# Beinsezii/skrample

Hardware: AMD Instinct MI355X
Metric: sampler steps/sec (fused DPM-2 SDE step, eps-pred, Karras sigmas, Bx4x128x128 bf16) + achieved HBM GB/s (higher is better)
Workload: dtype f32; 1 GPU; DPM order-2 SDE (eta=1) + Karras(Scaled) sigmas, eps-pred, B=256x4x128x128 bf16 latents per GPU (BASELINE north-star shape; cfg2 at 4x batch), in-kernel Philox noise, one fused launch per step; global_batch=256, per_gpu_batch=256, latent_dtype=bf16, compute_dtype=f32 registers, fp64 host coefficients, schedule_steps=20, buffer_sets=7, buffer_set_bytes=167772160, precondition_steps=3000, parallelism=batch-shard x1, no collective

## Files before the change

include/skrample_hip.h:

```cpp
#ifndef SKRAMPLE_HIP_H
#define SKRAMPLE_HIP_H

#include <stdint.h>

#ifdef __cplusplus
extern "C" {
#endif

#define SKR_ABI_VERSION 15
#define SKR_MAX_TERMS 80


enum skr_status {
  SKR_OK = 0,
  SKR_ERR_NULL = 1,
  SKR_ERR_DTYPE = 2,
  SKR_ERR_TERMS = 3,
  SKR_ERR_ALIGN = 4,
  SKR_ERR_SHAPE = 5,
  SKR_ERR_LAUNCH = 6,
  SKR_ERR_UNSUPPORTED = 7,
  SKR_ERR_LIBRARY = 8,
  SKR_ERR_CAPTURE = 9,
};

enum skr_dtype { SKR_BF16 = 0, SKR_F16 = 1, SKR_F32 = 2, SKR_F64 = 3, SKR_NONE = -1 };

typedef struct skr_step_plan {
  int32_t n_terms;
  int32_t n_group_a;
  int32_t dtype_a;
  int32_t dtype_b;
  int32_t out0_dtype;
  int32_t out1_dtype;
  int32_t acc_f64;
  int32_t noise_mode;
  double coef0[SKR_MAX_TERMS];
  double coef1[SKR_MAX_TERMS];
  double chain;
  double zeta0, zeta1;
  uint64_t stream0, stream1;
  int64_t sample_numel;
// ... 289 lines not shown
```

skrample_amd/_hip.py:

```python

from __future__ import annotations

import ctypes
import operator
import os
import sys
import threading

import torch

MAX_TERMS = 80
ABI_VERSION = 15
SKR_ERR_UNSUPPORTED = 7

BF16, F16, F32, F64, NONE = 0, 1, 2, 3, -1
DTYPE_CODE = {torch.bfloat16: BF16, torch.float16: F16, torch.float32: F32, torch.float64: F64}
CODE_DTYPE = {v: k for k, v in DTYPE_CODE.items()}

LIB_NAME = "libskrample_hip.so"
LIB_PATH = os.environ.get("SKR_HIP_LIB") or os.path.join(os.path.dirname(os.path.abspath(__file__)), "csrc", LIB_NAME)

EXPORTS = (
    "skr_step_launch",
    "skr_step_launch_indexed",
    "skr_step_launch_indexed_per_sample",
    "skr_step_launch_rolling",
    "skr_step_launch_channels_last",
    "skr_step_launch_masked",
# ... 689 lines not shown
```

skrample_amd/csrc/skr_step.hip:

```cpp


#include "skr_device.h"
#include "skr_step_common.h"
#include <new>

namespace skr {

Tuning g_tune;

template <typename T, typename Acc, bool HAS1, int N, int UV, bool TILE>
__device__ __forceinline__ void acc_batch(const StepArgs<Acc>& a, int k, int64_t v0, int64_t vhi, Acc s0[UV][VEC], Acc s1[UV][VEC]) {
  Raw<T> raw[UV][N];
#pragma unroll
  for (int u = 0; u < UV; ++u) {
    const int64_t v = v0 + u * BLOCK;
    if (v < vhi) {
#pragma unroll
      for (int j = 0; j < N; ++j) raw[u][j] = load_raw<T, TILE>(a.in[k + j], v);
    }
  }
#pragma unroll
  for (int u = 0; u < UV; ++u) {
    if (v0 + u * BLOCK >= vhi) continue;
#pragma unroll
// ... 226 lines not shown
        s1[i] = fma_(a.c1[1], ov[i], fma_(a.c1[0], sv[i], 0.f));
      }
#pragma unroll
      for (int j = 2; j < K; ++j) {
        float w[VEC];
        widen<T, float>(raw[u][j], w);
        const float c = a.c1[j];
#pragma unroll
        for (int i = 0; i < VEC; ++i) s1[i] = fma_(c, w[i], s1[i]);
      }
#pragma unroll
      for (int i = 0; i < VEC; ++i) s1[i] = fma_(a.chain, d[i], s1[i]);
      store8<T, float, TILE>(a.out1, v, s1);
      store8<T, float, TILE>(a.out0, v, d);
    }
  }
}


struct Geometry { dim3 grid; int mode; };

template <int UV, bool NOISE>
static Geometry geometry(int64_t numel, int64_t sample_numel) {
  const int64_t nvec = numel / VEC, per_block = BLOCK * UV;
  const bool aligned = (sample_numel % VEC) == 0;
  const int64_t vps = sample_numel / VEC, batch = numel / sample_numel;
  if (NOISE && aligned && vps >= per_block / 2 && batch <= 65535ll * 65535ll) {
    int64_t bx = (vps + per_block - 1) / per_block;
    if (bx > 65535) bx = 65535;
    const int64_t gy = batch < 65535 ? batch : 65535;
// ... 61 lines not shown
  Geometry g = geometry<UV, false>(args.numel, args.sample_numel);
  RkArgs ra;
  fill_operands(args.in, args.c1, args.n_terms, ra.in, ra.c1);
  ra.out0 = args.out0; ra.out1 = args.out1; ra.chain = args.chain;
  for (int i = 0; i < 4; ++i) ra.ck[i] = (float)args.ck[i];
  ra.conv_to = args.conv_to; ra.conv_from = args.conv_from; ra.numel = args.numel;
  return with_tile<sizeof(T) == 4>(args.numel, args.sample_numel, false, g.mode, [&](auto tile) {
    with_count<2, 8>(args.n_terms, [&](auto n) {
      hipLaunchKernelGGL((step_kernel_rk<T, decltype(n)::value, UV, decltype(tile)::value>), g.grid, dim3(BLOCK), 0, stream, ra);
    });
    return finish_launch();
  });
}

template <typename T>
static int launch_rk(const StepArgs<float>& args, hipStream_t stream) {
  {
    bool taken = false;
    const int rc = launch_one_trip_rk<T>(args, false, stream, taken);
    if (taken) return rc;
  }
  if (has_table(args.form)) return SKR_ERR_UNSUPPORTED;
  const int uv = g_tune.rk_uv ? g_tune.rk_uv : 1;
  if (uv == 4) return launch_rk_uv<T, 4>(args, stream);
  if (uv == 2) return launch_rk_uv<T, 2>(args, stream);
  return launch_rk_uv<T, 1>(args, stream);
}

template <typename TA, typename TB, typename TO0, typename TO1, typename Acc, bool ST0, bool HAS1, bool NOISE, bool CONV>
static int launch(StepArgs<Acc>& args, hipStream_t stream) {
  if constexpr (std::is_same<Acc, float>::value && std::is_same<TA, TB>::value && std::is_same<TO0, TA>::value && ST0 && !HAS1 && !CONV) {
    if (args.n_a == args.n_terms && (!NOISE || args.zeta0 != 0.f || has_table(args.form))) {
      bool taken = false;
      const int rc = launch_k<TA, NOISE>(args, stream, taken);
      if (taken) return rc;
    }
  }
  if constexpr (std::is_same<Acc, float>::value && std::is_same<TA, TB>::value && std::is_same<TO0, TA>::value && std::is_same<TO1, TA>::value && ST0 && HAS1 && CONV) {
    if (args.n_terms >= 2 && args.n_terms <= 8 && args.numel % VEC == 0) {
      if constexpr (!NOISE) return launch_rk<TA>(args, stream);
      else {
        bool taken = false;
        const int rc = launch_one_trip_rk<TA>(args, true, stream, taken);
        if (taken) return rc;
      }
    }
  }
  if constexpr (std::is_same<Acc, float>::value && sizeof(TA) == 2 && (std::is_same<TB, TA>::value || std::is_same<TB, float>::value) &&
                std::is_same<TO0, float>::value && std::is_same<TO1, TA>::value && ST0 && HAS1 && !CONV) {
    bool taken = false;
    const int rc = launch_one_trip_two<TA>(args, NOISE, std::is_same<TB, float>::value, stream, taken);
    if (taken) return rc;
  }
  if (has_table(args.form)) return SKR_ERR_UNSUPPORTED;
  constexpr int UV = uv_for(NOISE, HAS1);
  Geometry g = geometry<UV, NOISE>(args.numel, args.sample_numel);
  args.grid_mode = g.mode;
  args.vps = args.sample_numel / VEC;
  constexpr bool HAS32 = std::is_same<Acc, float>::value && (std::is_same<TA, float>::value || std::is_same<TB, float>::value ||
                                                               (ST0 && std::is_same<TO0, float>::value) || (HAS1 && std::is_same<TO1, float>::value));
  return with_tile<HAS32>(args.numel, args.sample_numel, NOISE, g.mode, [&](auto tile) {
    hipLaunchKernelGGL((step_kernel<TA, TB, TO0, TO1, Acc, ST0, HAS1, NOISE, CONV, decltype(tile)::value>), g.grid, dim3(BLOCK), 0, stream, args);
// ... 43 lines not shown
    a.c1[k] = (Acc)p.coef1[k];
  }
  for (int k = p.n_terms; k < MAXK; ++k) { a.in[k] = nullptr; a.c0[k] = 0; a.c1[k] = 0; }
  a.out0 = out0; a.out1 = out1; a.seeds = seeds;
  a.chain = (Acc)p.chain; a.zeta0 = (Acc)p.zeta0; a.zeta1 = (Acc)p.zeta1;
  a.stream0 = p.stream0; a.stream1 = p.stream1;
  a.numel = numel;
  a.sample_numel = p.sample_numel > 0 ? p.sample_numel : (numel > 0 ? numel : 1);
  a.inv_sample_numel = 1.0 / (double)a.sample_numel;
  a.n_a = p.n_group_a; a.n_terms = p.n_terms;
  a.conv_to = p.convert_to; a.conv_from = p.convert_from;
  for (int i = 0; i < 4; ++i) a.ck[i] = p.convert_k[i];
  if (a.conv_to != 0 || a.conv_from != 0) {
    for (int k = 0; k < p.n_terms; ++k) a.c0[k] = 0;
  }
  return pick<Acc>(a, p, s);
}

}

using skr::aligned16;

static int samples_ok(const skr_step_plan& p, int64_t numel, int64_t multiple) {
  if (p.sample_numel <= 0 || numel % p.sample_numel != 0) return SKR_ERR_SHAPE;
  return p.sample_numel % multiple == 0 ? SKR_OK : SKR_ERR_UNSUPPORTED;
}

static int validate_plan(const skr_step_plan& p, int64_t numel) {
  if (p.n_terms < 0 || p.n_terms > SKR_MAX_TERMS || p.n_group_a < 0 || p.n_group_a > p.n_terms) return SKR_ERR_TERMS;
  if (numel < 0) return SKR_ERR_SHAPE;
  if (p.out0_dtype == SKR_NONE && p.out1_dtype == SKR_NONE) return SKR_ERR_NULL;
  if (p.noise_mode != 0 && p.noise_mode != 1) return SKR_ERR_UNSUPPORTED;
  if (p.convert_to < 0 || p.convert_to > 3 || p.convert_from < 0 || p.convert_from > 3) return SKR_ERR_UNSUPPORTED;
  if ((p.convert_to || p.convert_from) && (p.n_group_a < 2 || p.out1_dtype == SKR_NONE)) return SKR_ERR_TERMS;
  if (skr::plan_draws(p) && numel > 0) return samples_ok(p, numel, 8);
  return SKR_OK;
}

int skr::step_launch_checks(const skr_step_plan* plan, const void* const* inputs, void* out0, void* out1, const uint64_t* seeds_dev, int64_t numel,
                            skr::RowForm form, const skr_step_row* rows, const int32_t* index, bool& empty) {
  empty = false;
  if (!plan || (has_table(form) && (!rows || (per_sample_rows(form) && !index)))) return SKR_ERR_NULL;
  const skr_step_plan& p = *plan;
  if (p.noise_mode == 1 && (has_table(form) || skr::plan_draws(p)) && numel > 0 && !seeds_dev) return SKR_ERR_NULL;
  if (const int rc = validate_plan(p, numel)) return rc;
  if (numel == 0) { empty = true; return SKR_OK; }
  const bool st0 = p.out0_dtype != SKR_NONE, has1 = p.out1_dtype != SKR_NONE;
  if ((p.n_terms > 0 && !inputs) || (st0 && !out0) || (has1 && !out1)) return SKR_ERR_NULL;
  if (const int rc = skr::check_ptrs(inputs, p.n_terms)) return rc;
// ... 3 lines not shown

static int step_launch_impl(const skr_step_plan* plan, const void* const* inputs, void* out0, void* out1, const uint64_t* seeds_dev, int64_t numel,
                            void* stream, skr::RowForm form, const skr_step_row* rows, const int32_t* index, int32_t row_offset) {
  skr::DeviceGuard device_guard(out0 ? out0 : out1);
  bool empty = false;
  if (const int rc = skr::step_launch_checks(plan, inputs, out0, out1, seeds_dev, numel, form, rows, index, empty)) return rc;
  if (empty) return SKR_OK;
  const skr_step_plan& p = *plan;
  hipStream_t s = reinterpret_cast<hipStream_t>(stream);
  if (has_table(form)) {
    const bool ragged = skr::ragged_launch(p, numel, form);
    if (per_sample_rows(form) || p.noise_mode == 1) {
      const int rc = samples_ok(p, numel, per_sample_rows(form) ? 2048 : 8);
      if (rc != SKR_OK && !(ragged && rc == SKR_ERR_UNSUPPORTED)) return rc;
    }
    if (p.acc_f64 || p.n_terms > SKR_ROW_TERMS || row_offset < 0) return SKR_ERR_UNSUPPORTED;
    if (ragged) return skr::launch_ragged(p, inputs, out0, seeds_dev, numel, s, form, rows, index, row_offset);
    return skr::run<float>(p, inputs, out0, out1, seeds_dev, numel, s, form, rows, index, row_offset);
  }
  return p.acc_f64 ? skr::run<double>(p, inputs, out0, out1, seeds_dev, numel, s)
                   : skr::run<float>(p, inputs, out0, out1, seeds_dev, numel, s);
}

extern "C" int skr_step_launch(const skr_step_plan* plan, const void* const* inputs, void* out0, void* out1,
                               const uint64_t* seeds_dev, int64_t numel, void* stream) {
  return step_launch_impl(plan, inputs, out0, out1, seeds_dev, numel, stream, skr::RowForm::Kernarg, nullptr, nullptr, 0);
}

extern "C" int skr_step_launch_indexed(const skr_step_plan* plan, const void* const* inputs, void* out0, void* out1,
                                       const uint64_t* seeds_dev, int64_t numel, const skr_step_row* rows_dev,
                                       const int32_t* index_dev, int32_t row_offset, void* stream) {
// ... 72 lines not shown
```

skrample_amd/csrc/skr_step_common.h:

```cpp
#pragma once
#include <hip/hip_runtime.h>
#include <stdlib.h>
#include <stdint.h>
#include <string.h>
#include <type_traits>
#include "../../include/skrample_hip.h"
#include "skr_philox.h"
#include "skr_pack.h"
#include "skr_launch.h"

namespace skr {

struct Tuning {
  int one_trip, xmap, tile, rk_uv, two_out, pace, rk_blk, two_nt, tape_words;
  Tuning() {
    const char* e;
    one_trip = !((e = getenv("SKR_ONE_TRIP")) && e[0] == '0');
    xmap = (e = getenv("SKR_XMAP")) ? atoi(e) : 7;
    tile = getenv("SKR_NO_TILE") == nullptr;
    rk_uv = (e = getenv("SKR_RK_UV")) ? atoi(e) : 0;
    two_out = getenv("SKR_NO_TWO_OUT") == nullptr;
    pace = getenv("SKR_NO_PACE") == nullptr;
    two_nt = (e = getenv("SKR_TWO_NT")) ? atoi(e) : -1;
    rk_blk = (e = getenv("SKR_RK_BLK")) ? atoi(e) : 0;
// ... 336 lines not shown
__device__ __forceinline__ void fma_noise8(Acc zeta, const float z[VEC], Acc s[VEC]) {
#pragma unroll
  for (int i = 0; i < VEC; ++i) s[i] = fma_(zeta, (Acc)z[i], s[i]);
}

struct RkArgs {
  const void* in[8];
  float c1[8];
  void* out0;
  void* out1;
  float chain;
  float ck[4];
  int32_t conv_to, conv_from;
  int64_t numel;
};

__device__ __forceinline__ uint32_t chunk_of(uint32_t b, int lr) {
  const uint32_t g = 3 + lr;
  return ((b >> g) << g) + ((b & 7u) << lr) + ((b >> 3) & ((1u << lr) - 1u));
}

static inline int xmap_lr_for(int64_t chunks) {
  int lr = g_tune.xmap;
  if (lr < 0) lr = 0;
  if (lr > 20) lr = 20;
  while (lr > 0 && chunks % (8ll << lr) != 0) --lr;
  return lr;
}

extern thread_local int g_last_hip_error;
// ... 40 lines not shown
```

skrample_amd/csrc/skr_step_fast.hip:

```cpp
#include "skr_step_common.h"

namespace skr {

template <int KMAX>
struct OneTripArgs {
  const void* in[KMAX];
  void* out0;
  const uint64_t* seeds;
  int32_t xmap_lr;
  int32_t bps_shift;
  uint64_t stream0;
  float c0[KMAX];
  float zeta0;
  RowRef tab;
};



template <bool PER_SAMPLE>
__device__ __forceinline__ const skr_step_row* row_at(const RowRef& r, uint32_t c, int32_t bps_shift) {
  if constexpr (PER_SAMPLE) {
    const uint32_t smp = (c >> (bps_shift < 0 ? 0 : bps_shift)) / (bps_shift < 0 ? (uint32_t)(-bps_shift) : 1u);
    return r.rows + ((r.index != nullptr ? r.index[__builtin_amdgcn_readfirstlane(smp)] : 0) + r.row_offset);
  } else {
// ... 252 lines not shown
  for (int j = 2; j < K; ++j) {
    if constexpr (F == RowForm::Rolling) { if (!on[j]) continue; }
    float w[VEC];
    widen<T, float>(raw[j], w);
    const float cj = cf[j];
#pragma unroll
    for (int i = 0; i < VEC; ++i) s1[i] = fma_(cj, w[i], s1[i]);
  }
#pragma unroll
  for (int i = 0; i < VEC; ++i) s1[i] = fma_(chain, d[i], s1[i]);
  if constexpr (NOISE) { if (n1) fma_noise8<float>(zeta1, z1, s1); }
  store8<T, float, TILE>(a.out1, v, s1);
  store8<T, float, TILE>(a.out0, v, d);
}

static bool one_trip_ok(int64_t numel, int64_t sample_numel, bool noise, RowForm form, int* bps_shift) {
  constexpr int64_t CHUNK = (int64_t)BLOCK * VEC;
  if ((!g_tune.one_trip && !has_table(form)) || numel % CHUNK != 0 || numel / CHUNK > 0x7fffffffll) return false;
  *bps_shift = 0;
  if (!noise && !per_sample_rows(form)) return true;
  if (sample_numel % CHUNK != 0) return false;
  const int64_t bps = sample_numel / CHUNK;
  if (bps > 0x3fffffffll) return false;
  *bps_shift = bps_shift_of(bps);
  return true;
}
template <typename T> static bool tile_switched_off(RowForm form) { return sizeof(T) == 4 && !g_tune.tile && !has_table(form); }

template <typename T, bool PACED, bool TABLE, typename Fn>
static bool with_form(RowForm form, Fn&& f) {
// ... 52 lines not shown
  with_count<2, 8>(args.n_terms, [&](auto n) {
    constexpr int N = decltype(n)::value;
    RkOneTripArgs<(N <= 4 ? 4 : 8)> ra;
    fill_operands(args.in, args.c1, N, ra.in, ra.c1);
    ra.seeds = args.seeds; ra.zeta1 = args.zeta1; ra.stream1 = args.stream1; ra.bps_shift = bps_shift;
    ra.out0 = args.out0; ra.out1 = args.out1; ra.chain = args.chain;
    for (int i = 0; i < 4; ++i) ra.ck[i] = (float)args.ck[i];
    ra.conv_to = args.conv_to; ra.conv_from = args.conv_from; ra.xmap_lr = xmap_lr_for(chunks); ra.tab = RowRef{args.rows, args.index, args.row_offset};
    with_form<T, false, true>(args.form, [&](auto tt, auto, auto fm) {
      hipLaunchKernelGGL((step_kernel_rk1<typename decltype(tt)::type, N, TILE, NOISE, decltype(fm)::value, BLK>), dim3(chunks), dim3(BLK), 0, stream, ra);
    });
  });
  return finish_launch();
}

template <typename T>
int launch_one_trip_rk(const StepArgs<float>& args, bool noise, hipStream_t stream, bool& taken) {
  taken = false;
  int bps_shift = 0;
  if (!one_trip_ok(args.numel, args.sample_numel, noise, args.form, &bps_shift) || tile_switched_off<T>(args.form)) return SKR_OK;
  if (noise && !has_table(args.form) && args.zeta0 != 0.f) return SKR_OK;
  taken = true;
  const unsigned chunks = (unsigned)(args.numel / ((int64_t)BLOCK * VEC));
  const bool small_blocks = g_tune.rk_blk == 128 || (g_tune.rk_blk == 0 && args.n_terms <= 6);
  if (small_blocks && chunks < 0x40000000u && bps_shift > -0x20000000)
    return noise ? launch_rk1<T, true, 128>(args, chunks, bps_shift, stream) : launch_rk1<T, false, 128>(args, chunks, bps_shift, stream);
  return noise ? launch_rk1<T, true, 256>(args, chunks, bps_shift, stream) : launch_rk1<T, false, 256>(args, chunks, bps_shift, stream);
}
template int launch_one_trip_rk<bf16_t>(const StepArgs<float>&, bool, hipStream_t, bool&);
template int launch_one_trip_rk<f16_t>(const StepArgs<float>&, bool, hipStream_t, bool&);
template int launch_one_trip_rk<float>(const StepArgs<float>&, bool, hipStream_t, bool&);

template <int NMAX>
struct TwoOutArgs {
  const void* in[NMAX];
  void* out0;
  void* out1;
  const uint64_t* seeds;
// ... 222 lines not shown
```

skrample_amd/diffusers.py:

```python

from __future__ import annotations

import abc
import contextlib
import ctypes
import dataclasses
import functools
import math
import weakref
from collections import OrderedDict
from collections.abc import Hashable, Mapping, Sequence
from types import MappingProxyType
from typing import Any

import numpy as np
import torch
from torch import Tensor

from . import scheduling
from .common import DeltaPoint, MergeStrategy, Point, Step
from .pytorch.noise import SUBSTREAMS, BatchTensorNoise, HostRandomBatch, Offset, Pyramid, Random, TensorNoiseCommon, TensorNoiseProps
from . import _hip
from .sampling import functional, interface, lazy, models, program, tableaux, traits
from .sampling import structured as sampling
# ... 1060 lines not shown
    invert_prediction: bool = False
    fake_config: dict[str, Any] = dataclasses.field(default_factory=DEFAULT_FAKE_CONFIG.copy)
    prefetch_noise: bool = False
    "(not in the reference) see SkrampleWrapperScheduler.prefetch_noise: the next step's noise is drawn on a side stream during this step's stages (opt-in)"
    alias_history: bool | str = "auto"
    "(not in the reference) see SkrampleWrapperScheduler.alias_history; snapshots are per stage call"

    def __post_init__(self) -> None:
        super().__post_init__()
        self._index = 0
        self._derivatives: list = []
        self._sample = None
        self._last_noise = None
        self._rk_programs: dict = {}
        self._rk_programs_for = None
        self._schedule = self.schedule

    @abc.abstractmethod
    def functional_sampler(self): ...

    def functional_interface(self):
        return self.functional_sampler(), self._schedule, self.model

    @abc.abstractmethod
    def tableau(self) -> tableaux.Tableau: ...

    def adjust_steps(self, steps: int) -> int:
        return self.functional_interface()[0].adjust_steps(steps)

    @abc.abstractmethod
# ... 26 lines not shown
        return len(self.tableau().stages)

    @property
    def config(self) -> OrderedDict:
        return attr_dict(**self.fake_config)

    def set_begin_index(self, begin_index: int = 0) -> None:
        assert begin_index % self.order == 0, f"Expected {begin_index=} to be multiple of {self.order=}!"
        super().set_begin_index(begin_index)
        self.fake_config["begin_index"] = begin_index

    def set_timesteps(self, num_inference_steps=None, device=None, timesteps=None, sigmas=None, mu=None) -> None:
        self._index = 0
        self._derivatives.clear()
        self._sample = None
        self._alias_stamps = []
        self._alias_auto = None
        with contextlib.suppress(AttributeError):
            del self.all_points
        with contextlib.suppress(AttributeError):
            del self.schedule_np_trim
        with contextlib.suppress(AttributeError):
            del self.trim_indices
        self.schedule = self._schedule
        steps = self._resolve_steps(num_inference_steps, timesteps, sigmas)
        if steps is None:
            return
        self._steps = steps
        if self.allow_dynamic:
            self.schedule = _apply_dynamic(self.schedule, steps, mu)
        self._retire_noise_generator()
        self._forget_issued_timesteps()
        if device is not None:
            self._device = torch.device(device)

    def reset_run(self) -> None:
        self._index = 0
        self._derivatives, self._sample = [], None
        self._alias_stamps = []
        self._alias_auto = None
        self._noise_ahead = None
        self._drain_noise_ahead()
        if self._noise_generator is not None:
            self._noise_generator._draws = 0

    def _next_noise_step(self) -> Step | None:
        nxt = self._index // self.order + 1
        return Step.from_int(nxt, self._steps) if nxt < self._steps else None

    def scale_noise(self, sample: Tensor, timestep: Tensor, noise: Tensor) -> Tensor:
        idx = self._lookup(self.schedule_np[:, 0].tolist(), timestep, 0)
        return Point(*self.schedule_np[idx]).add_noise(sample, noise)

# ... 49 lines not shown
                live: dict[int, Tensor] = {}
                if self._sample is not None and isinstance(self._sample, Tensor):
                    live[id(self._sample)] = self._sample
                for form in self._derivatives:
                    if isinstance(form, Lin):
                        for leaf, _ in form.terms.values():
                            if isinstance(leaf, Tensor):
                                live[id(leaf)] = leaf
                known = {id(t): (t, ptr, ver) for t, ptr, ver in self._alias_stamps}
                self._alias_stamps = [known.get(i) or (t, t.data_ptr(), t._version) for i, t in live.items() if t.numel() > 0]
        result = self._step_stage(model_output, sample, generator, return_dict)
        self._issue_noise_ahead()
        return result

    def _step_stage(self, model_output: Tensor, sample: Tensor, generator, return_dict: bool):
        if self.compute_scale is None and isinstance(sample, Tensor) and isinstance(model_output, Tensor):
            from .sampling import native

            done = native.rk_step(self, model_output, sample, generator)
            if done is not None:
                return self._finish(done[0], done[1], model_output, return_dict)
            self._derivatives = [lift(d) if isinstance(d, Tensor) else d for d in self._derivatives]
        owner = (self.schedule, self._steps, self.sampler_order, self.stochasticity, self.model, self.derivative_transform, self.compute_scale, self.invert_prediction)
        if self._rk_programs_for != owner:
            self._rk_programs, self._rk_programs_for = {}, owner
        held = len(self._derivatives)
        key = (self._index, held, sample.dtype, model_output.dtype, tuple(sample.shape))
        recorded = lazy.grad_recorded(model_output, sample, self._sample, *(leaf for form in self._derivatives if isinstance(form, Lin) for leaf, _ in form.terms.values()))
        prog = self._rk_programs.get(key) if not recorded else False
        if prog:
            done = self._replay_stage(prog, model_output, sample, generator)
            if done is not None:
                return self._finish(done[0], done[1], model_output, return_dict)

        points = [*self.all_points, Point(0, 0, 1)]
        conv = None
        if self.derivative_transform:
            space = self.derivative_transform
            convert = models.ModelConvert(self.model, self.derivative_transform)
            rounded = convert.rounded_program(points[self._index], negate_output=self.invert_prediction)
            if rounded is not None and rounded[:2] != (0, 0):
                conv = lazy.RoundedConversion(sample, model_output, *rounded)
                derivative = conv.node()
            else:
                output = -Lin.leaf(model_output) if self.invert_prediction else lift(model_output)
                ws, wo = convert.weights_to(points[self._index])
# ... 16 lines not shown
            abs(self.all_points[self._index].timestep - clean.timestep) < 1e-8 or abs(self.all_points[self._index].sigma - clean.sigma) < 1e-8
        ):
            synthesised = True
            base = lift(sample if self._sample is None else self._sample)
            delta = DeltaPoint(points[i0], points[i1])
            synth = (form - base * space.gamma(delta)) / space.delta(delta)
            form = self._stage_form(sample, synth, space, points[i0], points[i1], points[self._index + 1], generator)
            self._index += 1

        tracing = prog is None and _hip.trace is None and isinstance(sample, Tensor) and sample.is_cuda and not synthesised
        if tracing:
            _hip.trace = []
        try:
            with lazy.compute_scale(self.compute_scale):
                if conv is not None:
                    converted, result = lazy.evaluate([conv, form], [None, model_output.dtype])
                    self._derivatives = [d.substitute(conv, converted) for d in self._derivatives]
                    pred = converted
                else:
                    result = lazy.evaluate([form], [model_output.dtype])[0]
                    pred = LazyTensor(derivative, model_output.dtype) if (self.derivative_transform or self.invert_prediction) else model_output
            if tracing:
                built = None
                if len(_hip.trace) == 1 and (conv is not None or pred is model_output):
                    built = self._build_stage_program(_hip.trace[0], sample, model_output, base_before, pending, conv is not None, finished=not self._derivatives and self._sample is None)
                self._rk_programs[(start_index, held, sample.dtype, model_output.dtype, tuple(sample.shape))] = built or False
        finally:
            if tracing:
                _hip.trace = None
        return self._finish(result, pred, model_output, return_dict)

    @staticmethod
    def _single_tensor(form):
        if isinstance(form, Lin) and len(form.terms) == 1:
            (leaf, c), = form.terms.values()
            if isinstance(leaf, Tensor) and c == 1.0:
                return leaf
        return None

    def _build_stage_program(self, entry, sample, model_output, base_before, pending, converted: bool, finished: bool):
        plan, inputs, out0, out1, seeds, numel = entry
        table: dict[int, tuple] = {}
        for j, d in enumerate(pending):
            t = self._single_tensor(d)
            if t is None:
# ... 8 lines not shown
        table[id(sample)] = ("x",)
        roles = []
        for t in inputs:
            if id(t) not in table:
                return None
            roles.append(table[id(t)])
        philox = plan.noise_mode == 1
        if philox:
            if not isinstance(noise, lazy.PhiloxNoise) or noise.seeds is not seeds:
                return None
            if (converted and plan.zeta0 != 0.0) or (not converted and plan.zeta1 != 0.0):
                return None
        return {
            "plan": plan, "roles": roles, "dtypes": [t.dtype for t in inputs], "numel": numel, "shape": tuple(sample.shape),
            "out_dtypes": (out0.dtype, out1.dtype if out1 is not None else None), "converted": converted, "finished": finished,
            "noise": "philox" if philox else ("tensor" if isinstance(noise, Tensor) else None), "ptrs": (ctypes.c_void_p * max(len(inputs), 1))(),
            "drawn": noise is not None,
        }

    def _replay_stage(self, prog: dict, model_output: Tensor, sample: Tensor, generator):
        pending = [self._single_tensor(d) for d in self._derivatives]
        if any(t is None for t in pending):
            return None
        def fits(t, dt) -> bool:
            return isinstance(t, Tensor) and t.dtype == dt and t.numel() == prog["numel"] and t.is_contiguous() and t.data_ptr() % 16 == 0

        for role, dt in zip(prog["roles"], prog["dtypes"]):
            kind = role[0]
            if kind != "n" and not fits(sample if kind == "x" else model_output if kind == "o" else self._sample if kind == "b" else pending[role[1]], dt):
                return None
        noise = None
        if prog["noise"] is not None or prog.get("drawn"):
            base = sample if self._sample is None else self._sample
            noise = self.get_step_noise(Step.from_int(self._index // self.order, self._steps), base, self.noise_type, self.noise_props, generator, self.compute_scale, lazy_ok=True)
            self._noise_wanted = (self._next_noise_step(), base)
        plan = prog["plan"]
        seeds_ptr = None
# ... 11 lines not shown
            else:
                plan.stream0 = noise.stream
            seeds_ptr = noise.seeds.data_ptr()
        ops = []
        for role, dt in zip(prog["roles"], prog["dtypes"]):
            kind = role[0]
            ops.append(sample if kind == "x" else model_output if kind == "o" else self._sample if kind == "b" else noise if kind == "n" else pending[role[1]])
        dev = sample.device
        out0 = lazy.empty_output(prog["shape"], prog["out_dtypes"][0], dev)
        out1 = lazy.empty_output(prog["shape"], prog["out_dtypes"][1], dev) if prog["out_dtypes"][1] is not None else None
        arr = prog["ptrs"]
        for i, t in enumerate(ops):
            arr[i] = t.data_ptr()
        status = _hip.step_launch_raw(plan, arr, out0.data_ptr(), out1.data_ptr() if out1 is not None else None, seeds_ptr, prog["numel"], torch.cuda.current_stream(dev).cuda_stream)
        _hip.check(status, "skr_step_launch")
        result = out1 if prog["converted"] else out0
        pred = out0 if prog["converted"] else model_output
        if prog["finished"]:
            self._derivatives, self._sample = [], None
        else:
            self._derivatives.append(Lin.leaf(pred))
            if self._sample is None:
                self._sample = sample
        self._index += 1
        return result, pred


def _rk_from_config(cls, config, schedule, subschedule, schedule_modifiers, schedule_props, subschedule_props, merge, model, invert_prediction, **fields):
    parsed = parse_diffusers_config(config=config, sampler=None, schedule=schedule)
    return cls(
# ... 101 lines not shown
```

skrample_amd/sampling/lazy.py:

```python

from __future__ import annotations

import contextvars
import ctypes
import math
import os
from typing import Any, Sequence

import torch

from .. import _hip
from .._hip import SkrampleHipError

NUMBER = (int, float)

_compute_dtype: contextvars.ContextVar = contextvars.ContextVar("skr_compute_dtype", default=None)


class compute_scale:

    def __init__(self, dtype):
        self.dtype = dtype

    def __enter__(self):
# ... 409 lines not shown
    return tuple(out)


def _prepare_keeping_layout(t: torch.Tensor) -> torch.Tensor:
    if t.data_ptr() % 16:
        t = t.clone(memory_format=torch.preserve_format)
    return t


def in_place_layout(tensors, shape, allowed: bool = True) -> "tuple[int, int] | None":
    if not (allowed and channels_last and _hip.indexed is None):
        return None
    return shared_layout(tensors, shape)


def evaluate(forms: Sequence[Lin], dtypes: Sequence[torch.dtype | None], acc_f64: bool | None = None) -> list[torch.Tensor]:
    if not 1 <= len(forms) <= 2:
        raise SkrampleHipError("evaluate() takes one or two forms")
    conv = forms[0] if isinstance(forms[0], RoundedConversion) else None
    if conv is not None:
        if len(forms) != 2:
            raise SkrampleHipError("a rounded conversion is stored alongside the form that consumes it")
        dtypes = [conv.dtype, dtypes[1]]
        forms = [conv, forms[1]]
        f0 = Lin({id(conv.sample): (conv.sample, 0.0), id(conv.output): (conv.output, 0.0)}, conv.shape, conv.device)
    else:
        f0 = forms[0].expanded()
    f1 = forms[1].expanded(keep=forms[0]) if len(forms) == 2 else None
    shape, device = f0.shape, f0.device
    numel = math.prod(shape)
    out_dtypes = [d if d is not None else (f.dtype if isinstance(f, RoundedConversion) else _default_dtype(f)) for d, f in zip(dtypes, forms)]
    if is_host(device) or (f1 is not None and is_host(f1.device)):
        return _host_evaluate(conv, f0, f1, out_dtypes, acc_f64)
# ... 15 lines not shown
    if layout is not None:
        plan.sample_numel = layout[0] * layout[1]
        out0 = empty_output(shape, out_dtypes[0], device, channels_last=True)
        out1 = empty_output(shape, out_dtypes[1], device, channels_last=True) if f1 is not None else None
        _hip.launch_step(plan, operands, out0, out1, seeds, numel, device, layout)
        return [out0] if out1 is None else [out0, out1]
    if torch.is_grad_enabled() and any(t.requires_grad for t in operands):
        if conv is not None:
            plan_a = conversion_gradient(conv.to_kind, conv.from_kind, conv.k)
        else:
            plan_a = None
        outs = _StepFunction.apply(plan, plan_a, seeds, shape, numel, device, *operands)
        return list(outs) if f1 is not None else [outs]
    out0 = empty_output(shape, out_dtypes[0], device)
    out1 = empty_output(shape, out_dtypes[1], device) if f1 is not None else None
    _hip.launch_step(plan, operands, out0, out1, seeds, numel, device)
    return [out0] if out1 is None else [out0, out1]


def _lower(conv, f0: "Lin", f1: "Lin | None", chain: float, out_dtypes, acc_f64: bool | None, fuse1: bool = True, max_terms: int = _hip.MAX_TERMS,
           keep_layout: bool = False):
    shape, numel = f0.shape, math.prod(f0.shape)
    tensors: dict[int, torch.Tensor] = {}
    c0: dict[int, float] = {}
    c1: dict[int, float] = {}
    noise0: list[tuple[PhiloxNoise, float]] = []
    noise1: list[tuple[PhiloxNoise, float]] = []
    for which, form in ((0, f0), (1, f1)):
        if form is None:
            continue
        for i, (leaf, c) in form.terms.items():
            if c == 0.0 and not (conv is not None and which == 0):
# ... 76 lines not shown
    if conv is not None:
        plan.convert_to, plan.convert_from = conv.to_kind, conv.from_kind
        for k in range(4):
            plan.convert_k[k] = conv.k[k]
    seeds = None
    if fused0 is not None or fused1 is not None:
        plan.noise_mode = 1
        src = fused0 or fused1
        seeds = src[0].seeds
        plan.sample_numel = src[0].sample_numel
        if fused0 is not None:
            plan.zeta0, plan.stream0 = fused0[1], fused0[0].stream
        if fused1 is not None:
            plan.zeta1, plan.stream1 = fused1[1], fused1[0].stream
    return plan, [prepared[i] for i in order], seeds


def mask_layout(mask_shape: Sequence[int], shape: Sequence[int]) -> tuple[int, int]:
    shape, mask_shape = tuple(shape), tuple(mask_shape)
    refuse = f"a mask of shape {mask_shape} does not broadcast over leading axes of {shape}"
    if len(shape) < 2 or not 1 <= len(mask_shape) <= len(shape):
        raise SkrampleHipError(refuse)
    full = (1,) * (len(shape) - len(mask_shape)) + mask_shape
    if full[0] not in (1, shape[0]):
        raise SkrampleHipError(f"{refuse}: its batch axis must be 1 or {shape[0]}")
    inner = 1
    while inner < len(shape) and full[inner] == 1:
        inner += 1
    if full[inner:] != shape[inner:]:
        raise SkrampleHipError(f"{refuse}: behind its leading 1s it must spell out {shape[inner:]}")
# ... 533 lines not shown
```

Measured before the change: 38760 steps/s.

## Rebuild RK stage input from prior stage terms instead of reading it

Adds a rebuild mode for Runge-Kutta stage launches. When the stage input is exactly the output of the previous fused launch, the kernel recomputes it in registers as a rounded linear combination of the previous launch's operands rather than reading it from HBM. The operands it needs are largely already loaded for the current stage, so the intent is to cut one full tensor read per stage. In exchange the host must track stage records, pointers and version stamps to stay bit-exact, and the code adds new kernel variants and a flag-bit ABI extension.

After: 38770 steps/s, median of 2. About the same (+0.0%).

```diff
diff --git a/include/skrample_hip.h b/include/skrample_hip.h
--- a/include/skrample_hip.h
+++ b/include/skrample_hip.h
@@ -26,6 +26,7 @@
 
 enum skr_dtype { SKR_BF16 = 0, SKR_F16 = 1, SKR_F32 = 2, SKR_F64 = 3, SKR_NONE = -1 };
 
+#define SKR_CONVERT_REBUILD 0x100
 typedef struct skr_step_plan {
   int32_t n_terms;
   int32_t n_group_a;
diff --git a/skrample_amd/_hip.py b/skrample_amd/_hip.py
--- a/skrample_amd/_hip.py
+++ b/skrample_amd/_hip.py
@@ -12,6 +12,7 @@
 MAX_TERMS = 80
 ABI_VERSION = 15
 SKR_ERR_UNSUPPORTED = 7
+CONVERT_REBUILD = 0x100
 
 BF16, F16, F32, F64, NONE = 0, 1, 2, 3, -1
 DTYPE_CODE = {torch.bfloat16: BF16, torch.float16: F16, torch.float32: F32, torch.float64: F64}
diff --git a/skrample_amd/csrc/skr_step.hip b/skrample_amd/csrc/skr_step.hip
--- a/skrample_amd/csrc/skr_step.hip
+++ b/skrample_amd/csrc/skr_step.hip
@@ -264,6 +264,53 @@
       store8<T, float, TILE>(a.out1, v, s1);
       store8<T, float, TILE>(a.out0, v, d);
     }
+  }
+}
+
+template <typename T, int K, bool TILE>
+__global__ __launch_bounds__(BLOCK) void step_kernel_rk_rebuild(const RkGridRebuildArgs a) {
+  const int64_t vhi = a.numel / VEC;
+  const int64_t stride = (int64_t)gridDim.x * BLOCK;
+  const float k[4] = {a.ck[0], a.ck[1], a.ck[2], a.ck[3]};
+  for (int64_t v = (int64_t)blockIdx.x * BLOCK + threadIdx.x; v < vhi; v += stride) {
+    Raw<T> raw[K];
+#pragma unroll
+    for (int j = 1; j < K; ++j) raw[j] = load_raw<T, TILE>(a.in[j], v);
+    float sv[VEC], ov[VEC], d[VEC], s1[VEC];
+#pragma unroll
+    for (int i = 0; i < VEC; ++i) sv[i] = fma_(0.f, 0.f, 0.f);
+#pragma unroll
+    for (int j = 2; j < K; ++j) {
+      float w[VEC];
+      widen<T, float>(raw[j], w);
+      const float pj = a.pc[j];
+#pragma unroll
+      for (int i = 0; i < VEC; ++i) sv[i] = fma_(pj, w[i], sv[i]);
+    }
+#pragma unroll
+    for (int i = 0; i < VEC; ++i) sv[i] = rnd<T>(sv[i]);
+    if constexpr (sizeof(T) == 2) {
+#pragma unroll
+      for (int j = 2; j < K; ++j) pin_raw(raw[j]);
+    }
+    widen<T, float>(raw[1], ov);
+#pragma unroll
+    for (int i = 0; i < VEC; ++i) {
+      d[i] = convert_rounded<T, float>(sv[i], ov[i], a.conv_to, a.conv_from, k);
+      s1[i] = fma_(a.c1[1], ov[i], fma_(a.c1[0], sv[i], 0.f));
+    }
+#pragma unroll
+    for (int j = 2; j < K; ++j) {
+      float w[VEC];
+      widen<T, float>(raw[j], w);
+      const float c = a.c1[j];
+#pragma unroll
+      for (int i = 0; i < VEC; ++i) s1[i] = fma_(c, w[i], s1[i]);
+    }
+#pragma unroll
+    for (int i = 0; i < VEC; ++i) s1[i] = fma_(a.chain, d[i], s1[i]);
+    store8<T, float, TILE>(a.out1, v, s1);
+    store8<T, float, TILE>(a.out0, v, d);
   }
 }
 
@@ -355,6 +402,23 @@
 }
 
 template <typename T>
+static int launch_rk_rebuild(const StepArgs<float>& args, hipStream_t stream) {
+  Geometry g = geometry<1, false>(args.numel, args.sample_numel);
+  RkGridRebuildArgs ra;
+  fill_operands(args.in, args.c1, args.n_terms, ra.in, ra.c1);
+  for (int k = 0; k < 8; ++k) ra.pc[k] = k < args.n_terms ? args.c0[k] : 0.f;
+  ra.out0 = args.out0; ra.out1 = args.out1; ra.chain = args.chain;
+  for (int i = 0; i < 4; ++i) ra.ck[i] = (float)args.ck[i];
+  ra.conv_to = args.conv_to & ~SKR_CONVERT_REBUILD; ra.conv_from = args.conv_from; ra.numel = args.numel;
+  return with_tile<sizeof(T) == 4>(args.numel, args.sample_numel, false, g.mode, [&](auto tile) {
+    with_count<3, 8>(args.n_terms, [&](auto n) {
+      hipLaunchKernelGGL((step_kernel_rk_rebuild<T, decltype(n)::value, decltype(tile)::value>), g.grid, dim3(BLOCK), 0, stream, ra);
+    });
+    return finish_launch();
+  });
+}
+
+template <typename T>
 static int launch_rk(const StepArgs<float>& args, hipStream_t stream) {
   {
     bool taken = false;
@@ -362,6 +426,7 @@
     if (taken) return rc;
   }
   if (has_table(args.form)) return SKR_ERR_UNSUPPORTED;
+  if (args.conv_to & SKR_CONVERT_REBUILD) return launch_rk_rebuild<T>(args, stream);
   const int uv = g_tune.rk_uv ? g_tune.rk_uv : 1;
   if (uv == 4) return launch_rk_uv<T, 4>(args, stream);
   if (uv == 2) return launch_rk_uv<T, 2>(args, stream);
@@ -387,6 +452,7 @@
       }
     }
   }
+  if (args.conv_to & SKR_CONVERT_REBUILD) return SKR_ERR_UNSUPPORTED;
   if constexpr (std::is_same<Acc, float>::value && sizeof(TA) == 2 && (std::is_same<TB, TA>::value || std::is_same<TB, float>::value) &&
                 std::is_same<TO0, float>::value && std::is_same<TO1, TA>::value && ST0 && HAS1 && !CONV) {
     bool taken = false;
@@ -460,6 +526,15 @@
   if (a.conv_to != 0 || a.conv_from != 0) {
     for (int k = 0; k < p.n_terms; ++k) a.c0[k] = 0;
   }
+  if (p.convert_to & SKR_CONVERT_REBUILD) {
+    for (int k = p.n_terms; k >= 1; --k) {
+      a.in[k] = inputs[k - 1];
+      a.c1[k] = (Acc)p.coef1[k - 1];
+      a.c0[k] = k >= 2 ? (Acc)p.coef0[k - 1] : (Acc)0;
+    }
+    a.in[0] = nullptr; a.c1[0] = (Acc)p.coef0[0]; a.c0[0] = 0;
+    a.n_a = a.n_terms = p.n_terms + 1;
+  }
   return pick<Acc>(a, p, s);
 }
 
@@ -477,8 +552,15 @@
   if (numel < 0) return SKR_ERR_SHAPE;
   if (p.out0_dtype == SKR_NONE && p.out1_dtype == SKR_NONE) return SKR_ERR_NULL;
   if (p.noise_mode != 0 && p.noise_mode != 1) return SKR_ERR_UNSUPPORTED;
-  if (p.convert_to < 0 || p.convert_to > 3 || p.convert_from < 0 || p.convert_from > 3) return SKR_ERR_UNSUPPORTED;
+  const int32_t to_kind = p.convert_to & ~SKR_CONVERT_REBUILD;
+  if (to_kind < 0 || to_kind > 3 || p.convert_from < 0 || p.convert_from > 3) return SKR_ERR_UNSUPPORTED;
   if ((p.convert_to || p.convert_from) && (p.n_group_a < 2 || p.out1_dtype == SKR_NONE)) return SKR_ERR_TERMS;
+  if (p.convert_to & SKR_CONVERT_REBUILD) {
+    const bool narrow = p.dtype_a == SKR_BF16 || p.dtype_a == SKR_F16 || p.dtype_a == SKR_F32;
+    if ((to_kind == 0 && p.convert_from == 0) || p.n_terms > 7 || p.n_group_a != p.n_terms || !narrow || p.out0_dtype != p.dtype_a ||
+        p.out1_dtype != p.dtype_a || p.acc_f64 || p.noise_mode != 0 || numel % 8 != 0)
+      return SKR_ERR_UNSUPPORTED;
+  }
   if (skr::plan_draws(p) && numel > 0) return samples_ok(p, numel, 8);
   return SKR_OK;
 }
@@ -512,7 +594,7 @@
       const int rc = samples_ok(p, numel, per_sample_rows(form) ? 2048 : 8);
       if (rc != SKR_OK && !(ragged && rc == SKR_ERR_UNSUPPORTED)) return rc;
     }
-    if (p.acc_f64 || p.n_terms > SKR_ROW_TERMS || row_offset < 0) return SKR_ERR_UNSUPPORTED;
+    if (p.acc_f64 || p.n_terms > SKR_ROW_TERMS || row_offset < 0 || (p.convert_to & SKR_CONVERT_REBUILD)) return SKR_ERR_UNSUPPORTED;
     if (ragged) return skr::launch_ragged(p, inputs, out0, seeds_dev, numel, s, form, rows, index, row_offset);
     return skr::run<float>(p, inputs, out0, out1, seeds_dev, numel, s, form, rows, index, row_offset);
   }
diff --git a/skrample_amd/csrc/skr_step_common.h b/skrample_amd/csrc/skr_step_common.h
--- a/skrample_amd/csrc/skr_step_common.h
+++ b/skrample_amd/csrc/skr_step_common.h
@@ -374,6 +374,7 @@
   int32_t conv_to, conv_from;
   int64_t numel;
 };
+struct RkGridRebuildArgs : RkArgs { float pc[8]; };
 
 __device__ __forceinline__ uint32_t chunk_of(uint32_t b, int lr) {
   const uint32_t g = 3 + lr;
diff --git a/skrample_amd/csrc/skr_step_fast.hip b/skrample_amd/csrc/skr_step_fast.hip
--- a/skrample_amd/csrc/skr_step_fast.hip
+++ b/skrample_amd/csrc/skr_step_fast.hip
@@ -290,6 +290,68 @@
   store8<T, float, TILE>(a.out0, v, d);
 }
 
+template <int KMAX>
+struct RkRebuildArgs {
+  const void* in[KMAX];
+  void* out0;
+  void* out1;
+  int32_t xmap_lr;
+  int32_t conv_to, conv_from;
+  float c1[KMAX];
+  float chain;
+  float ck[4];
+  float pc[KMAX];
+};
+
+template <typename T, int K, bool TILE, int BLK>
+__global__ __launch_bounds__(BLK) void step_kernel_rk1_rebuild(const RkRebuildArgs<(K <= 4 ? 4 : 8)> a) {
+  static_assert(K >= 3, "the stage input has at least one term");
+  const uint32_t c = chunk_of(blockIdx.x, a.xmap_lr);
+  const int64_t v = (int64_t)c * BLK + threadIdx.x;
+  Raw<T> raw[K];
+#pragma unroll
+  for (int j = 1; j < K; ++j) raw[j] = load_raw<T, TILE>(a.in[j], v);
+  __builtin_amdgcn_sched_barrier(0);
+  float k[4] = {a.ck[0], a.ck[1], a.ck[2], a.ck[3]}, cf[K], pc[K], chain = a.chain;
+#pragma unroll
+  for (int j = 0; j < K; ++j) { cf[j] = a.c1[j]; pc[j] = a.pc[j]; }
+  float sv[VEC], ov[VEC], d[VEC], s1[VEC];
+#pragma unroll
+  for (int i = 0; i < VEC; ++i) sv[i] = fma_(0.f, 0.f, 0.f);
+#pragma unroll
+  for (int j = 2; j < K; ++j) {
+    float w[VEC];
+    widen<T, float>(raw[j], w);
+    const float pj = pc[j];
+#pragma unroll
+    for (int i = 0; i < VEC; ++i) sv[i] = fma_(pj, w[i], sv[i]);
+  }
+#pragma unroll
+  for (int i = 0; i < VEC; ++i) sv[i] = rnd<T>(sv[i]);
+  if constexpr (sizeof(T) == 2) {
+#pragma unroll
+    for (int j = 2; j < K; ++j) pin_raw(raw[j]);
+  }
+  widen<T, float>(raw[1], ov);
+#pragma unroll
+  for (int i = 0; i < VEC; ++i) {
+    d[i] = convert_rounded<T, float>(sv[i], ov[i], a.conv_to, a.conv_from, k);
+    s1[i] = fma_(cf[1], ov[i], fma_(cf[0], sv[i], 0.f));
+  }
+#pragma unroll
+  for (int j = 2; j < K; ++j) {
+    float w[VEC];
+    widen<T, float>(raw[j], w);
+    const float cj = cf[j];
+#pragma unroll
+    for (int i = 0; i < VEC; ++i) s1[i] = fma_(cj, w[i], s1[i]);
+  }
+#pragma unroll
+  for (int i = 0; i < VEC; ++i) s1[i] = fma_(chain, d[i], s1[i]);
+  store8<T, float, TILE>(a.out1, v, s1);
+  store8<T, float, TILE>(a.out0, v, d);
+}
+
 static bool one_trip_ok(int64_t numel, int64_t sample_numel, bool noise, RowForm form, int* bps_shift) {
   constexpr int64_t CHUNK = (int64_t)BLOCK * VEC;
   if ((!g_tune.one_trip && !has_table(form)) || numel % CHUNK != 0 || numel / CHUNK > 0x7fffffffll) return false;
@@ -372,6 +434,25 @@
   return finish_launch();
 }
 
+template <typename T, int BLK>
+static int launch_rk1_rebuild(const StepArgs<float>& args, unsigned chunks, hipStream_t stream) {
+  constexpr bool TILE = sizeof(T) == 4;
+  if constexpr (BLK == 128) chunks *= 2;
+  bool launched = false;
+  with_count<3, 8>(args.n_terms, [&](auto n) {
+    constexpr int N = decltype(n)::value;
+    RkRebuildArgs<(N <= 4 ? 4 : 8)> ra;
+    fill_operands(args.in, args.c1, N, ra.in, ra.c1);
+    for (int k = 0; k < (N <= 4 ? 4 : 8); ++k) ra.pc[k] = k < N ? args.c0[k] : 0.f;
+    ra.out0 = args.out0; ra.out1 = args.out1; ra.chain = args.chain; ra.xmap_lr = xmap_lr_for(chunks);
+    for (int i = 0; i < 4; ++i) ra.ck[i] = (float)args.ck[i];
+    ra.conv_to = args.conv_to & ~SKR_CONVERT_REBUILD; ra.conv_from = args.conv_from;
+    hipLaunchKernelGGL((step_kernel_rk1_rebuild<T, N, TILE, BLK>), dim3(chunks), dim3(BLK), 0, stream, ra);
+    launched = true;
+  });
+  return launched ? finish_launch() : SKR_ERR_UNSUPPORTED;
+}
+
 template <typename T>
 int launch_one_trip_rk(const StepArgs<float>& args, bool noise, hipStream_t stream, bool& taken) {
   taken = false;
@@ -380,6 +461,11 @@
   if (noise && !has_table(args.form) && args.zeta0 != 0.f) return SKR_OK;
   taken = true;
   const unsigned chunks = (unsigned)(args.numel / ((int64_t)BLOCK * VEC));
+  if (args.conv_to & SKR_CONVERT_REBUILD) {
+    if (noise || has_table(args.form)) return SKR_ERR_UNSUPPORTED;
+    const bool small = g_tune.rk_blk == 128 || (g_tune.rk_blk == 0 && args.n_terms - 1 <= 6);
+    return small && chunks < 0x40000000u ? launch_rk1_rebuild<T, 128>(args, chunks, stream) : launch_rk1_rebuild<T, 256>(args, chunks, stream);
+  }
   const bool small_blocks = g_tune.rk_blk == 128 || (g_tune.rk_blk == 0 && args.n_terms <= 6);
   if (small_blocks && chunks < 0x40000000u && bps_shift > -0x20000000)
     return noise ? launch_rk1<T, true, 128>(args, chunks, bps_shift, stream) : launch_rk1<T, false, 128>(args, chunks, bps_shift, stream);
diff --git a/skrample_amd/diffusers.py b/skrample_amd/diffusers.py
--- a/skrample_amd/diffusers.py
+++ b/skrample_amd/diffusers.py
@@ -1098,6 +1098,7 @@
         self._last_noise = None
         self._rk_programs: dict = {}
         self._rk_programs_for = None
+        self._rk_link = lazy.StageLink()
         self._schedule = self.schedule
 
     @abc.abstractmethod
@@ -1154,6 +1155,7 @@
         self._index = 0
         self._derivatives.clear()
         self._sample = None
+        self._rk_link.prev = None
         self._alias_stamps = []
         self._alias_auto = None
         with contextlib.suppress(AttributeError):
@@ -1177,6 +1179,7 @@
     def reset_run(self) -> None:
         self._index = 0
         self._derivatives, self._sample = [], None
+        self._rk_link.prev = None
         self._alias_stamps = []
         self._alias_auto = None
         self._noise_ahead = None
@@ -1256,6 +1259,8 @@
         return result
 
     def _step_stage(self, model_output: Tensor, sample: Tensor, generator, return_dict: bool):
+        link = self._rk_link
+        handed, link.prev = link.prev, None
         if self.compute_scale is None and isinstance(sample, Tensor) and isinstance(model_output, Tensor):
             from .sampling import native
 
@@ -1271,7 +1276,7 @@
         recorded = lazy.grad_recorded(model_output, sample, self._sample, *(leaf for form in self._derivatives if isinstance(form, Lin) for leaf, _ in form.terms.values()))
         prog = self._rk_programs.get(key) if not recorded else False
         if prog:
-            done = self._replay_stage(prog, model_output, sample, generator)
+            done = self._replay_stage(prog, model_output, sample, generator, handed)
             if done is not None:
                 return self._finish(done[0], done[1], model_output, return_dict)
 
@@ -1318,7 +1323,8 @@
         try:
             with lazy.compute_scale(self.compute_scale):
                 if conv is not None:
-                    converted, result = lazy.evaluate([conv, form], [None, model_output.dtype])
+                    link.prev = handed
+                    converted, result = lazy.evaluate([conv, form], [None, model_output.dtype], link=link)
                     self._derivatives = [d.substitute(conv, converted) for d in self._derivatives]
                     pred = converted
                 else:
@@ -1333,6 +1339,18 @@
             if tracing:
                 _hip.trace = None
         return self._finish(result, pred, model_output, return_dict)
+
+    def _rebuild_holds(self, prog: dict, handed, model_output: Tensor, sample: Tensor, pending) -> bool:
+        if handed is None or not lazy.REBUILD_STAGES or _hip.indexed is not None:
+            return False
+        if sample is not handed.out1 or sample.data_ptr() != handed.ptr or sample._version != handed.version:
+            return False
+        plan = prog["plan"]
+        bound = [self._sample if role[0] == "b" else pending[role[1]] if role[0] == "d" else None for role in prog["roles"][1:]]
+        if prog["roles"][0][0] != "o" or len(bound) != len(handed.terms) or handed.dtype != plan.dtype_a:
+            return False
+        return all(t is b and c == plan.coef0[k] and (t.data_ptr(), t._version) == stamp
+                   for k, ((t, c), b, stamp) in enumerate(zip(handed.terms, bound, handed.stamps), start=1))
 
     @staticmethod
     def _single_tensor(form):
@@ -1371,13 +1389,16 @@
         return {
             "plan": plan, "roles": roles, "dtypes": [t.dtype for t in inputs], "numel": numel, "shape": tuple(sample.shape),
             "out_dtypes": (out0.dtype, out1.dtype if out1 is not None else None), "converted": converted, "finished": finished,
+            "rebuilt": bool(plan.convert_to & _hip.CONVERT_REBUILD),
             "noise": "philox" if philox else ("tensor" if isinstance(noise, Tensor) else None), "ptrs": (ctypes.c_void_p * max(len(inputs), 1))(),
             "drawn": noise is not None,
         }
 
-    def _replay_stage(self, prog: dict, model_output: Tensor, sample: Tensor, generator):
+    def _replay_stage(self, prog: dict, model_output: Tensor, sample: Tensor, generator, handed=None):
         pending = [self._single_tensor(d) for d in self._derivatives]
         if any(t is None for t in pending):
+            return None
+        if prog["rebuilt"] and not self._rebuild_holds(prog, handed, model_output, sample, pending):
             return None
         def fits(t, dt) -> bool:
             return isinstance(t, Tensor) and t.dtype == dt and t.numel() == prog["numel"] and t.is_contiguous() and t.data_ptr() % 16 == 0
@@ -1419,6 +1440,8 @@
             arr[i] = t.data_ptr()
         status = _hip.step_launch_raw(plan, arr, out0.data_ptr(), out1.data_ptr() if out1 is not None else None, seeds_ptr, prog["numel"], torch.cuda.current_stream(dev).cuda_stream)
         _hip.check(status, "skr_step_launch")
+        if prog["converted"]:
+            self._rk_link.prev = lazy.StageRecord.of(plan, ops, out0, out1)
         result = out1 if prog["converted"] else out0
         pred = out0 if prog["converted"] else model_output
         if prog["finished"]:
diff --git a/skrample_amd/sampling/lazy.py b/skrample_amd/sampling/lazy.py
--- a/skrample_amd/sampling/lazy.py
+++ b/skrample_amd/sampling/lazy.py
@@ -447,9 +447,12 @@
     return shared_layout(tensors, shape)
 
 
-def evaluate(forms: Sequence[Lin], dtypes: Sequence[torch.dtype | None], acc_f64: bool | None = None) -> list[torch.Tensor]:
+def evaluate(forms: Sequence[Lin], dtypes: Sequence[torch.dtype | None], acc_f64: bool | None = None, link: "StageLink | None" = None) -> list[torch.Tensor]:
     if not 1 <= len(forms) <= 2:
         raise SkrampleHipError("evaluate() takes one or two forms")
+    prev = None
+    if link is not None:
+        prev, link.prev = link.prev, None
     conv = forms[0] if isinstance(forms[0], RoundedConversion) else None
     if conv is not None:
         if len(forms) != 2:
@@ -495,8 +498,24 @@
         return list(outs) if f1 is not None else [outs]
     out0 = empty_output(shape, out_dtypes[0], device)
     out1 = empty_output(shape, out_dtypes[1], device) if f1 is not None else None
+    if link is not None and REBUILD_STAGES and _hip.indexed is None:
+        plan, operands = rebuilt_stage(plan, operands, prev) or (plan, operands)
     _hip.launch_step(plan, operands, out0, out1, seeds, numel, device)
+    if link is not None:
+        link.prev = StageRecord.of(plan, operands, out0, out1)
     return [out0] if out1 is None else [out0, out1]
+
+
+REBUILD_STAGES = True
+"False: every Runge-Kutta stage launch reads its stage input (the reading launch is the reference the rebuilding one is held to, bit for bit)"
+
+
+class StageLink:
+
+    __slots__ = ("prev",)
+
+    def __init__(self):
+        self.prev = None
 
 
 def _lower(conv, f0: "Lin", f1: "Lin | None", chain: float, out_dtypes, acc_f64: bool | None, fuse1: bool = True, max_terms: int = _hip.MAX_TERMS,
@@ -603,6 +622,62 @@
         if fused1 is not None:
             plan.zeta1, plan.stream1 = fused1[1], fused1[0].stream
     return plan, [prepared[i] for i in order], seeds
+
+
+class StageRecord:
+
+    __slots__ = ("out1", "ptr", "version", "dtype", "terms", "stamps")
+
+    def __init__(self, out1: torch.Tensor, dtype: int, terms: list):
+        self.out1, self.ptr, self.version, self.dtype, self.terms = out1, out1.data_ptr(), out1._version, dtype, terms
+        self.stamps = [(t.data_ptr(), t._version) for t, _ in terms]
+
+    @classmethod
+    def of(cls, plan, operands, out0, out1) -> "StageRecord | None":
+        rebuilt = bool(plan.convert_to & _hip.CONVERT_REBUILD)
+        if not (plan.convert_to or plan.convert_from) or out0 is None or out1 is None:
+            return None
+        if plan.n_group_a != plan.n_terms or plan.dtype_a not in (_hip.BF16, _hip.F16, _hip.F32) or plan.out0_dtype != plan.dtype_a or plan.out1_dtype != plan.dtype_a:
+            return None
+        if plan.acc_f64 or plan.noise_mode != 0:
+            return None
+        if rebuilt:
+            if plan.coef0[0] != 0.0 or plan.coef1[0] != 0.0:
+                return None
+            summed = [(operands[k], plan.coef1[k]) for k in range(1, plan.n_terms)]
+        else:
+            if plan.coef1[1] != 0.0:
+                return None
+            summed = [(operands[0], plan.coef1[0])] + [(operands[k], plan.coef1[k]) for k in range(2, plan.n_terms)]
+        return cls(out1, plan.dtype_a, [(t, float(c)) for t, c in summed if c != 0.0] + [(out0, float(plan.chain))])
+
+
+def rebuilt_stage(plan, operands, prev: "StageRecord | None"):
+    if prev is None or not (plan.convert_to or plan.convert_from) or plan.convert_to & _hip.CONVERT_REBUILD or plan.n_terms < 2:
+        return None
+    sample = operands[0]
+    if sample is not prev.out1 or sample.data_ptr() != prev.ptr or sample._version != prev.version:
+        return None
+    if plan.n_group_a != plan.n_terms or plan.dtype_a != prev.dtype or plan.out0_dtype != plan.dtype_a or plan.out1_dtype != plan.dtype_a or plan.acc_f64 or plan.noise_mode != 0:
+        return None
+    terms = prev.terms
+    if not 1 <= len(terms) <= 6 or 1 + len(terms) >= plan.n_terms or any(t.dtype != sample.dtype or t.shape != sample.shape for t, _ in terms):
+        return None
+    if any((t.data_ptr(), t._version) != stamp for (t, _), stamp in zip(terms, prev.stamps)):
+        return None
+    mine = {id(t): plan.coef1[k] for k, t in enumerate(operands) if k >= 2}
+    at = [next((i for i, (t, _) in enumerate(terms) if t is op), -1) for op in operands[2:]]
+    if -1 in at or at != sorted(at) or len(set(at)) != len(at):
+        return None
+    out = _hip.StepPlanC.from_buffer_copy(plan)
+    out.n_terms = out.n_group_a = 1 + len(terms)
+    out.convert_to = plan.convert_to | _hip.CONVERT_REBUILD
+    for k in range(_hip.MAX_TERMS):
+        out.coef0[k] = out.coef1[k] = 0.0
+    out.coef0[0], out.coef1[0] = plan.coef1[0], plan.coef1[1]
+    for k, (t, c) in enumerate(terms, start=1):
+        out.coef0[k], out.coef1[k] = c, mine.get(id(t), 0.0)
+    return out, [operands[1], *(t for t, _ in terms)]
 
 
 def mask_layout(mask_shape: Sequence[int], shape: Sequence[int]) -> tuple[int, int]:
```
